# MachinaIO/mxx

Hardware: AMD Instinct MI355X
Metric: dcrt_ring_ops_per_s (higher is better)
Workload: dtype u32

## Files before the change

mxx_amd/csrc/arith.hip:

```cpp
#include "matmul_tile.h"

#include <algorithm>
#include <vector>

enum { OP_ADD = 0, OP_SUB = 1, OP_MUL = 2, OP_NEG = 3 };

template <typename W, int OP, bool BCAST, int VN>
__global__ void elementwise_kernel(W *__restrict__ out, const W *__restrict__ a, const W *__restrict__ b,
                                   const LimbConst *__restrict__ limbs, uint32_t L, uint32_t logN,
                                   size_t words_per_poly, size_t total_vecs) {
    size_t v = static_cast<size_t>(blockIdx.x) * blockDim.x + threadIdx.x;
    const size_t stride = static_cast<size_t>(gridDim.x) * blockDim.x;
    for (; v < total_vecs; v += stride) {
        const size_t w0 = v * VN;
        const uint32_t limb = static_cast<uint32_t>((w0 >> logN) % L);
        const LimbConst lc = limbs[limb];
        const W q = static_cast<W>(lc.q);
        const size_t bw0 = BCAST ? (w0 % words_per_poly) : w0;
        W av[VN], bv[VN], ov[VN];
        if (VN == 1) {
            av[0] = a[w0];
            bv[0] = b[bw0];
        } else {
            typedef typename std::conditional<sizeof(W) == 4, uint4, ulonglong2>::type V16;
// ... 322 lines not shown
        if (pending + kMmKC > lazy) {
            pending = 0;
#pragma unroll
            for (int i = 0; i < 8; ++i)
#pragma unroll
                for (int j = 0; j < 8; ++j) acc[i][j] = reduce_u64_sum(acc[i][j], q, lc.mu64);
        }
        if (ch + 1 < nchunks) stage(buf ^ 1);
        __syncthreads();
    }
#pragma unroll
    for (int i = 0; i < 8; ++i) {
        const uint32_t r = r0 + wr * 8 + i;
        if (r >= rows) continue;
#pragma unroll
        for (int j = 0; j < 8; ++j) {
            const uint32_t c = c0 + wc * 8 + j;
            if (c >= cols) continue;
            C[(static_cast<size_t>(r) * cols + c) * polyw + base] = reduce_u64_sum(acc[i][j], q, lc.mu64);
        }
    }
}

static int launch_matmul_lds_u32(GpuMatrix *out, const GpuMatrix *lhs, const GpuMatrix *rhs) {
    GpuContext *ctx = out->ctx;
    const uint32_t rows = static_cast<uint32_t>(lhs->rows), inner = static_cast<uint32_t>(lhs->cols),
                   cols = static_cast<uint32_t>(rhs->cols);
    const uint32_t L = static_cast<uint32_t>(matrix_limbs(out)), N = static_cast<uint32_t>(ctx->N);
    const uint32_t row_tiles = (rows + 15) / 16, col_tiles = (cols + 15) / 16, slot_chunks = N / 64;
    const uint64_t groups = static_cast<uint64_t>(L) * slot_chunks;
    const uint64_t blocks = groups * row_tiles * col_tiles;
    if (blocks > 0x7fffffffull) return set_error("gpu_matrix_mul: matrix too large");
    const uint32_t remap = (groups % 8 == 0) ? 1u : 0u;
    ctx->last_kernel = "matmul_lds_kernel_u32 (64 slots x 16x16 tile, operands staged through registers into LDS)";
    MXX_LAUNCH(matmul_lds_kernel_u32, dim3(static_cast<unsigned>(blocks)), dim3(256), 0, ctx->stream,
                       static_cast<uint32_t *>(words_ptr(out)), static_cast<const uint32_t *>(words_ptr(lhs)),
                       static_cast<const uint32_t *>(words_ptr(rhs)), ctx->d_limbs, rows, inner, cols, L, N, row_tiles,
                       col_tiles, slot_chunks, remap);
    HIP_TRY(hipGetLastError());
    return 0;
}

template <typename W, int TR, int TC, int SV, bool PF = false>
static int launch_matmul_cfg(GpuMatrix *out, const GpuMatrix *lhs, const GpuMatrix *rhs) {
    GpuContext *ctx = out->ctx;
    const uint32_t rows = static_cast<uint32_t>(lhs->rows), inner = static_cast<uint32_t>(lhs->cols),
                   cols = static_cast<uint32_t>(rhs->cols);
    const uint32_t L = static_cast<uint32_t>(matrix_limbs(out)), N = static_cast<uint32_t>(ctx->N);
    if (!tile_grid_fits(rows, cols, TR, TC)) return set_error("gpu_matrix_mul: matrix too large");
    const TileGrid g = tile_grid<TR, TC, SV>(ctx, rows, cols, L, rhs->bytes);
    const bool nt = g.streamed;
    auto label = [](bool nt_, int pk) {
        return std::string("matmul_kernel<") + (sizeof(W) == 4 ? "u32," : "u64,") + std::to_string(TR) + "," + std::to_string(TC) + "," +
               std::to_string(SV) + (PF ? ",loads-ahead" : "") + (nt_ ? ",nt" : "") +
               (pk == 2 ? ",packed24 B" : pk == 1 ? ",packed24 A" : "") +
               "> (register tile rows x cols x slots per lane" + (nt_ ? ", B streamed once with non-temporal loads" : "") +
               (pk ? ", 3-byte residues" : "") + ")";
    };
    static const std::string name[2][3] = {{label(false, 0), label(false, 1), label(false, 2)}, {label(true, 0), label(true, 1), label(true, 2)}};
    W *c = static_cast<W *>(words_ptr(out));
#define MXX_MM(NT, PK) \
    MXX_LAUNCH((matmul_kernel<W, TR, TC, SV, PF, NT, PK>), g.grid, dim3(g.threads), 0, ctx->stream, c, a, b, ctx->d_limbs, rows, inner, cols, L, N, g.col_tiles)
    if constexpr (sizeof(W) == 4 && SV == 4) {
        if (lhs->ctx == ctx && rhs->ctx == ctx) {
            if (lhs->layout.v.load(std::memory_order_acquire) == GPU_MATRIX_LAYOUT_PACKED24 &&
                rhs->layout.v.load(std::memory_order_acquire) == GPU_MATRIX_LAYOUT_PACKED24)
                (void)words_ptr(lhs);
            std::lock_guard<std::mutex> lk(ctx->layout_mutex);
            bool pa = false, pb = false;
            const W *a = static_cast<const W *>(packed24_ptr(lhs, &pa)), *b = static_cast<const W *>(packed24_ptr(rhs, &pb));
            if (pa && pb) return set_error("gpu_matrix_mul: both operands packed");
            const int pk = (pa ? 1 : 0) | (pb ? 2 : 0);
            ctx->last_kernel = name[nt ? 1 : 0][pk].c_str();
            switch (pk | (nt ? 4 : 0)) {
                case 0: MXX_MM(false, 0); break;
                case 1: MXX_MM(false, 1); break;
                case 2: MXX_MM(false, 2); break;
                case 4: MXX_MM(true, 0); break;
                case 5: MXX_MM(true, 1); break;
                default: MXX_MM(true, 2); break;
            }
            HIP_TRY(hipGetLastError());
            return 0;
        }
    }
    const W *a = static_cast<const W *>(words_ptr(lhs)), *b = static_cast<const W *>(words_ptr(rhs));
    ctx->last_kernel = name[nt ? 1 : 0][0].c_str();
    if (nt) MXX_MM(true, 0);
    else MXX_MM(false, 0);
#undef MXX_MM
    HIP_TRY(hipGetLastError());
    return 0;
}

int launch_matmul(GpuMatrix *out, const GpuMatrix *lhs, const GpuMatrix *rhs) {
    GpuContext *ctx = out->ctx;
    const size_t rows = lhs->rows, cols = rhs->cols;
    const int N = ctx->N;
    if (ctx->wide)
        return dispatch_stacked_tile(ctx, stacked_tile(ctx, rows, cols, matrix_limbs(out)), [&](auto cfg) {
            typedef decltype(cfg) T;
            return launch_matmul_cfg<typename T::W, T::TR, T::TC, T::SV>(out, lhs, rhs);
        });
    {
        const char force = ctx->env.matmul_path;
        const bool lds_ok = N >= 64 && (N % 64) == 0;
        const bool want_mfma = force ? (force == 'm') : false;
        if (want_mfma) {
            const int rc = launch_matmul_mfma_u32(out, lhs, rhs);
            if (rc >= 0) return rc;
        }
        const size_t inner = lhs->cols;
        const bool narrow = cols < 16 && inner < 128;
        const bool rows32 = !narrow && rows >= 24 && (rows % 32 == 0 || rows % 32 >= 24);
        const bool want_wide = force ? (force == 'w') : (rows32 && cols >= 32 && ((cols + 31) / 32) * 2 <= (cols + 15) / 16);
        if (want_wide) {
            const int rc = launch_matmul_dma32_u32(out, lhs, rhs);
            if (rc >= 0) return rc;
        }
        const bool want_dma = force ? (force == 'd' || force == 'w') : (rows32 && cols >= 16);
        if (want_dma) {
            const int rc = launch_matmul_dma_u32(out, lhs, rhs);
            if (rc >= 0) return rc;
        }
        const uint64_t lds_blocks = static_cast<uint64_t>(matrix_limbs(out)) * (N / 64) * ((cols + 15) / 16);
        const bool thin = rows <= 2 && cols >= 8 &&
                          lds_blocks <= 512 && (inner >= 128 || (rows >= 2 && inner >= 64));
        const bool want_lds = force ? (force == 'l' || force == 'd' || force == 'w') : ((rows >= 9 && cols >= 8 && !narrow) || thin);
        if (lds_ok && want_lds) return launch_matmul_lds_u32(out, lhs, rhs);
    }
    if (N >= 4) {
        switch (ctx->env.matmul_tile) {
#define MXX_TILE(R, C, S)                                                                   \
    case (R * 100 + C * 10 + S) * 2: return launch_matmul_cfg<uint32_t, R, C, S>(out, lhs, rhs); \
    case (R * 100 + C * 10 + S) * 2 + 1: return launch_matmul_cfg<uint32_t, R, C, S, true>(out, lhs, rhs);
            MXX_TILE(1, 8, 4) MXX_TILE(1, 4, 4) MXX_TILE(2, 8, 4) MXX_TILE(2, 4, 4) MXX_TILE(3, 4, 4) MXX_TILE(4, 4, 4)
            MXX_TILE(3, 8, 2) MXX_TILE(4, 8, 1) MXX_TILE(8, 8, 1) MXX_TILE(4, 8, 2)
#undef MXX_TILE
            default: break;
        }
        if (rows > 4 && rows <= 8) return launch_matmul_cfg<uint32_t, 8, 8, 1>(out, lhs, rhs);
        if (rows >= 4) {
            const uint64_t waves4 = static_cast<uint64_t>((N + 63) / 64) * ((cols + 7) / 8) * matrix_limbs(out);
            return waves4 <= 8192 ? launch_matmul_cfg<uint32_t, 4, 8, 1, true>(out, lhs, rhs) : launch_matmul_cfg<uint32_t, 4, 8, 1>(out, lhs, rhs);
        }
        if (rows == 3) {
            const uint64_t waves3 = static_cast<uint64_t>((N / 4 + 63) / 64) * ((cols + 3) / 4) * matrix_limbs(out);
            return waves3 <= 4096 ? launch_matmul_cfg<uint32_t, 3, 4, 4, true>(out, lhs, rhs) : launch_matmul_cfg<uint32_t, 3, 4, 4>(out, lhs, rhs);
        }
        const uint32_t tc = (rows >= 2 || cols >= 8) ? 8 : 4;
        const uint64_t tile_waves = static_cast<uint64_t>((N / 4 + 63) / 64) * ((rows + 1) / 2) * ((cols + tc - 1) / tc) * matrix_limbs(out);
        const bool ahead = tile_waves <= (rows >= 2 ? 1024u : 8192u);
        if (rows >= 2) return ahead ? launch_matmul_cfg<uint32_t, 2, 8, 4, true>(out, lhs, rhs) : launch_matmul_cfg<uint32_t, 2, 8, 4>(out, lhs, rhs);
        if (cols >= 8) return ahead ? launch_matmul_cfg<uint32_t, 1, 8, 4, true>(out, lhs, rhs) : launch_matmul_cfg<uint32_t, 1, 8, 4>(out, lhs, rhs);
        return ahead ? launch_matmul_cfg<uint32_t, 1, 4, 4, true>(out, lhs, rhs) : launch_matmul_cfg<uint32_t, 1, 4, 4>(out, lhs, rhs);
    }
    return launch_matmul_cfg<uint32_t, 1, 4, 1>(out, lhs, rhs);
}

template <typename W, int OP, bool BCAST>
static int launch_elementwise_typed(GpuMatrix *out, const GpuMatrix *a, const GpuMatrix *b) {
    GpuContext *ctx = out->ctx;
    const size_t words = matrix_words(out);
    if (words == 0) return 0;
    const size_t wpp = matrix_limbs(out) * static_cast<size_t>(ctx->N);
    const uint32_t L = static_cast<uint32_t>(matrix_limbs(out));
    constexpr int VNATIVE = 16 / sizeof(W);
    MXX_TRACE_BYTES(static_cast<double>(words) * sizeof(W) * (1 + (OP == OP_NEG || BCAST || a == b ? 1 : 2)));
    if (ctx->N >= VNATIVE) {
        const size_t vecs = words / VNATIVE;
        unsigned blocks = static_cast<unsigned>(std::min<size_t>((vecs + 255) / 256, 16384));
        MXX_LAUNCH((elementwise_kernel<W, OP, BCAST, VNATIVE>), dim3(blocks), dim3(256), 0, ctx->stream,
                           static_cast<W *>(words_ptr(out)), static_cast<const W *>(words_ptr(a)),
                           static_cast<const W *>(words_ptr(b)), ctx->d_limbs, L, ctx->logN, wpp, vecs);
    } else {
        unsigned blocks = static_cast<unsigned>(std::min<size_t>((words + 255) / 256, 16384));
        MXX_LAUNCH((elementwise_kernel<W, OP, BCAST, 1>), dim3(blocks), dim3(256), 0, ctx->stream,
                           static_cast<W *>(words_ptr(out)), static_cast<const W *>(words_ptr(a)),
                           static_cast<const W *>(words_ptr(b)), ctx->d_limbs, L, ctx->logN, wpp, words);
    }
    HIP_TRY(hipGetLastError());
    return 0;
}

template <int OP, bool BCAST>
static int launch_elementwise(GpuMatrix *out, const GpuMatrix *a, const GpuMatrix *b) {
    if (ctx_activate(out->ctx)) return 1;
    return out->ctx->wide ? launch_elementwise_typed<uint64_t, OP, BCAST>(out, a, b)
                          : launch_elementwise_typed<uint32_t, OP, BCAST>(out, a, b);
}

static GpuMatrix matrix_view(const GpuMatrix *m, size_t first_poly, size_t rows, size_t cols, size_t poly_bytes) {
    GpuMatrix v;
    v.ctx = m->ctx;
    v.level = m->level;
    v.rows = rows;
    v.cols = cols;
    v.format = m->format;
    v.storage = static_cast<char *>(words_ptr(m)) + first_poly * poly_bytes;
    v.bytes = rows * cols * poly_bytes;
    return v;
}

extern "C" int gpupoly_matrix_add_rows(GpuMatrix *out, size_t dst_row, const GpuMatrix *lhs, const GpuMatrix *rhs) {
    ABI_GUARD_BEGIN
    if (!out || !lhs || !rhs) return set_error("gpupoly_matrix_add_rows: null matrix");
    if (matrix_check_same_shape(lhs, rhs, "gpupoly_matrix_add_rows")) return 1;
    if (out->ctx != lhs->ctx || out->level != lhs->level) return set_error("gpupoly_matrix_add_rows: context/level mismatch");
    if (out->cols != lhs->cols || dst_row > out->rows || lhs->rows > out->rows - dst_row)
        return set_error("gpupoly_matrix_add_rows: row block out of range");
    if (lhs->format != rhs->format) return set_error("gpupoly_matrix_add_rows: operands must share a format");
    if (row_block_overlaps(out, dst_row, lhs->rows, lhs) || row_block_overlaps(out, dst_row, lhs->rows, rhs))
        return set_error("gpupoly_matrix_add_rows: output must not alias an input");
    const size_t poly_bytes = matrix_limbs(out) * static_cast<size_t>(out->ctx->N) * out->ctx->word_bytes;
    GpuMatrix view = matrix_view(out, dst_row * out->cols, lhs->rows, lhs->cols, poly_bytes);
    int rc = launch_elementwise<OP_ADD, false>(&view, lhs, rhs);
    if (rc) return rc;
    out->format = lhs->format;
    return 0;
    ABI_GUARD_END
}

extern "C" int gpupoly_matrix_ntt_add_rows(GpuMatrix *out, size_t dst_row, GpuMatrix *coeff, const GpuMatrix *addend,
                                           int consume_coeff) {
    ABI_GUARD_BEGIN
    if (!out || !coeff || !addend) return set_error("gpupoly_matrix_ntt_add_rows: null matrix");
    if (matrix_check_same_shape(coeff, addend, "gpupoly_matrix_ntt_add_rows")) return 1;
    if (out->ctx != coeff->ctx || out->level != coeff->level) return set_error("gpupoly_matrix_ntt_add_rows: context/level mismatch");
    if (out->cols != coeff->cols || dst_row > out->rows || coeff->rows > out->rows - dst_row)
        return set_error("gpupoly_matrix_ntt_add_rows: row block out of range");
    if (coeff->format != GPU_POLY_FORMAT_COEFF || addend->format != GPU_POLY_FORMAT_EVAL)
        return set_error("gpupoly_matrix_ntt_add_rows: expects a COEFF matrix and an EVAL addend");
    if (row_block_overlaps(out, dst_row, coeff->rows, coeff) || row_block_overlaps(out, dst_row, coeff->rows, addend))
        return set_error("gpupoly_matrix_ntt_add_rows: output must not alias an input");
    GpuContext *ctx = out->ctx;
    out->format = GPU_POLY_FORMAT_EVAL;
    const size_t polys = matrix_polys(coeff);
    if (polys == 0) return 0;
    if (ctx_activate(ctx)) return 1;
    const size_t L = matrix_limbs(out);
    const size_t poly_bytes = L * static_cast<size_t>(ctx->N) * ctx->word_bytes;
    GpuMatrix view = matrix_view(out, dst_row * out->cols, coeff->rows, coeff->cols, poly_bytes);
    view.format = GPU_POLY_FORMAT_EVAL;
    if (!ctx->wide) {
        const int rc = launch_ntt_add_u32(ctx, static_cast<uint32_t *>(words_ptr(&view)), static_cast<const uint32_t *>(words_ptr(coeff)),
                                          static_cast<const uint32_t *>(words_ptr(addend)), polys * L, static_cast<uint32_t>(L));
        if (rc >= 0) return rc;
    }
    if (consume_coeff) {
        int rc = launch_ntt(ctx, words_ptr(coeff), polys * L, static_cast<int>(L), false);
        if (rc) return rc;
        coeff->format = GPU_POLY_FORMAT_EVAL;
        return launch_elementwise<OP_ADD, false>(&view, coeff, addend);
    }
    MXX_TRACED_COPY("copy (device to device)", ctx->stream, 2.0 * view.bytes,
                    HIP_TRY(hipMemcpyAsync(words_ptr(&view), words_ptr(coeff), view.bytes, hipMemcpyDeviceToDevice, ctx->stream)));
    int rc = launch_ntt(ctx, words_ptr(&view), polys * L, static_cast<int>(L), false);
    if (rc) return rc;
    return launch_elementwise<OP_ADD, false>(&view, &view, addend);
    ABI_GUARD_END
}

extern "C" int gpu_matrix_add(GpuMatrix *out, const GpuMatrix *lhs, const GpuMatrix *rhs) {
    ABI_GUARD_BEGIN
    if (matrix_check_same_shape(out, lhs, "gpu_matrix_add") || matrix_check_same_shape(lhs, rhs, "gpu_matrix_add"))
        return 1;
    if (partial_overlap(out, lhs) || partial_overlap(out, rhs))
        return set_error("gpu_matrix_add: the output overlaps an operand without being the same block");
    int rc = launch_elementwise<OP_ADD, false>(out, lhs, rhs);
    if (rc) return rc;
    out->format = rhs->format;
    return 0;
    ABI_GUARD_END
}

extern "C" int gpu_matrix_sub(GpuMatrix *out, const GpuMatrix *lhs, const GpuMatrix *rhs) {
    ABI_GUARD_BEGIN
    if (matrix_check_same_shape(out, lhs, "gpu_matrix_sub") || matrix_check_same_shape(lhs, rhs, "gpu_matrix_sub"))
        return 1;
    if (partial_overlap(out, lhs) || partial_overlap(out, rhs))
        return set_error("gpu_matrix_sub: the output overlaps an operand without being the same block");
    int rc = launch_elementwise<OP_SUB, false>(out, lhs, rhs);
    if (rc) return rc;
    out->format = rhs->format;
    return 0;
    ABI_GUARD_END
}

extern "C" int gpupoly_matrix_neg(GpuMatrix *out, const GpuMatrix *src) {
    ABI_GUARD_BEGIN
    if (matrix_check_same_shape(out, src, "gpupoly_matrix_neg")) return 1;
    if (partial_overlap(out, src))
        return set_error("gpupoly_matrix_neg: the output overlaps the source without being the same block");
    int rc = launch_elementwise<OP_NEG, false>(out, src, src);
    if (rc) return rc;
    out->format = src->format;
    return 0;
    ABI_GUARD_END
}

extern "C" int gpu_matrix_mul_scalar(GpuMatrix *out, const GpuMatrix *lhs, const GpuMatrix *scalar) {
    ABI_GUARD_BEGIN
    if (!scalar) return set_error("gpu_matrix_mul_scalar: null scalar");
    if (matrix_check_same_shape(out, lhs, "gpu_matrix_mul_scalar")) return 1;
    if (scalar->ctx != lhs->ctx || scalar->level != lhs->level)
        return set_error("gpu_matrix_mul_scalar: context/level mismatch");
// ... 501 lines not shown
```

mxx_amd/csrc/common.h:

```cpp
#pragma once

#include <hip/hip_runtime.h>

#include <atomic>
#include <cstddef>
#include <cstdint>
#include <cstdio>
#include <exception>
#include <map>
#include <unordered_map>
#include <mutex>
#include <string>
#include <vector>

#include "../../include/gpupoly.h"

constexpr size_t GPUPOLY_MAX_LIMBS = 64;

struct LimbConst {
    uint64_t q;
    uint64_t mu;
    uint64_t mu64;
    uint64_t n_inv;
    uint64_t n_inv_sh;
    uint64_t mu32;
    uint64_t inv_last_w;
    uint64_t inv_last_w_sh;
    uint32_t kbits;
    uint32_t lazy_terms;
};

struct EnvSwitches {
    int ntt_path = 0;
    int ntt14 = 0;
    bool decompose_fused = true;
    char matmul_path = 0;
    int matmul_tile = 0;
    bool gsamp_simple = false;
    bool gsamp_no_uni = false;
    bool p1_simple = false;
    int sampler_per_lane = 0;
    int sampler_fill_every = 0;
    bool ntt64_int = false;
    int ntt_phase = 0;
    bool serde_general = false;
    bool rng_compat = false;
    bool pack24 = true;
    size_t mul_decompose_many_budget = 0;
    size_t gadget_scalar_budget = 0;
    char mul_sum_path = 0;
    void load();
};

struct GpuContext {
    EnvSwitches env;
    int device = 0;
    std::vector<int> gpu_ids;
    uint32_t logN = 0;
    int N = 0;
    int level = 0;
    uint32_t dnum = 0;
    int limb_count = 0;
    bool wide = false;
    int word_bytes = 4;
    uint32_t crt_bits = 0;
    std::vector<uint64_t> moduli;
    hipStream_t stream = nullptr;
    LimbConst *d_limbs = nullptr;
    LimbConst *d_limbs_r = nullptr;
    void *d_tw_fwd = nullptr;
    void *d_tw_fwd_sh = nullptr;
    void *d_tw_inv = nullptr;
    void *d_tw_inv_sh = nullptr;
    void *d_tw2_fwd = nullptr;
    void *d_tw2_inv = nullptr;
    bool lazy_ok = false;
    bool tight_ok = false;
    void *d_tw2s_inv = nullptr;
    bool signed_ok = false;
    void *d_twf_fwd = nullptr, *d_twf_inv = nullptr;
    void *d_flimbs = nullptr;
    bool f64_ok = false;
    uint64_t *d_garner = nullptr;
    std::vector<uint64_t> garner_inv;
    std::vector<LimbConst> limbs;
    hipEvent_t timer_start = nullptr, timer_stop = nullptr;
    std::vector<hipEvent_t> marks;
    std::mutex mutex;
    bool pool_ok = false;
    std::mutex alloc_mutex;
    std::multimap<size_t, void *> free_blocks;
    std::unordered_map<void *, size_t> live_blocks;
    size_t cached_bytes = 0, cache_limit = 0;
    std::atomic<const char *> last_kernel{""};
    bool pack24_ok = false;
    std::mutex layout_mutex;
    std::map<uint32_t, void *> gadget_weights;
    std::map<std::vector<uint64_t>, void *> gadget_const_tables;
};

struct LayoutTag {
    std::atomic<int> v{GPU_MATRIX_LAYOUT_WORDS};
    LayoutTag() = default;
    LayoutTag(const LayoutTag &o) : v(o.v.load(std::memory_order_acquire)) {}
    LayoutTag &operator=(const LayoutTag &o) {
        v.store(o.v.load(std::memory_order_acquire), std::memory_order_release);
        return *this;
    }
};

struct GpuMatrix {
    GpuContext *ctx = nullptr;
    int level = 0;
    size_t rows = 0, cols = 0;
    int format = GPU_POLY_FORMAT_EVAL;
    void *storage = nullptr;
    size_t bytes = 0;
    LayoutTag layout;
    bool borrowed = false;
    GpuMatrix *parent = nullptr;
    int views = 0;
};

struct GpuEventSet {
    std::vector<hipEvent_t> events;
    int device = 0;
    void *staging = nullptr;
    GpuContext *ctx = nullptr;
    void *dev_staging = nullptr;
};

struct GpuP1CovarianceCache {
    GpuContext *ctx = nullptr;
    int level = 0;
    size_t d = 0, m = 0, n = 0;
    double sigma = 0, s = 0, dgg_stddev = 0;
    double *sqrt_var = nullptr;
    double *update_coeff = nullptr;
    void *karney_div = nullptr;
};

static inline dim3 item_grid(size_t items, unsigned threads) {
    const size_t blocks = (items + threads - 1) / threads;
    const size_t max_x = (static_cast<size_t>(1) << 31) / threads;
    if (blocks <= max_x) return dim3(static_cast<unsigned>(blocks ? blocks : 1));
    const size_t y = (blocks + max_x - 1) / max_x;
    return dim3(static_cast<unsigned>((blocks + y - 1) / y), static_cast<unsigned>(y));
}
#if defined(__HIPCC__)
__device__ __forceinline__ size_t item_index() {
    return (static_cast<size_t>(blockIdx.y) * gridDim.x + blockIdx.x) * blockDim.x + threadIdx.x;
}
#endif

extern std::atomic<uint64_t> g_kernel_launches;
extern std::atomic<int> g_trace_on;
void trace_launch_begin(const char *name, hipStream_t stream, dim3 grid, dim3 block);
void trace_launch_end(hipStream_t stream);
void trace_set_bytes(double bytes);
#define MXX_TRACE_BYTES(b)                                                                        \
    do {                                                                                          \
        if (g_trace_on.load(std::memory_order_relaxed)) trace_set_bytes(static_cast<double>(b)); \
    } while (0)
#define MXX_LAUNCH(kern, grid, block, lds, strm, ...)                          \
    do {                                                                       \
        g_kernel_launches.fetch_add(1, std::memory_order_relaxed);             \
        const bool mxx_tr_ = g_trace_on.load(std::memory_order_relaxed) != 0;  \
        if (mxx_tr_) trace_launch_begin(#kern, strm, grid, block);             \
        hipLaunchKernelGGL(kern, grid, block, lds, strm, __VA_ARGS__);         \
        if (mxx_tr_) trace_launch_end(strm);                                   \
    } while (0)
#define MXX_TRACED_COPY(name, strm, bytes, stmt)                               \
    do {                                                                       \
        const bool mxx_tr_ = g_trace_on.load(std::memory_order_relaxed) != 0;  \
        if (mxx_tr_) {                                                         \
            trace_set_bytes(static_cast<double>(bytes));                       \
            trace_launch_begin(name, strm, dim3(0), dim3(0));                  \
        }                                                                      \
        stmt;                                                                  \
        if (mxx_tr_) trace_launch_end(strm);                                   \
    } while (0)

int set_error(const char *msg);
int set_error(const std::string &msg);
int set_error(hipError_t err, const char *what);

#define HIP_TRY(expr)                                          \
    do {                                                       \
        hipError_t _e = (expr);                                \
        if (_e != hipSuccess) return set_error(_e, #expr);     \
    } while (0)

extern int (*g_roctx_push)(const char *);
extern int (*g_roctx_pop)();
void roctx_init_once();
struct RoctxScope {
    bool on;
    explicit RoctxScope(const char *name) {
        roctx_init_once();
        on = g_roctx_push != nullptr;
        if (on) g_roctx_push(name);
    }
    ~RoctxScope() {
        if (on) g_roctx_pop();
    }
};

#define ABI_GUARD_BEGIN try { RoctxScope roctx_scope_(__func__);
#define ABI_GUARD_END                                                         \
    }                                                                         \
    catch (const std::exception &e) { return set_error(e.what()); }           \
    catch (...) { return set_error("unknown exception in libgpupoly"); }

inline size_t matrix_polys(const GpuMatrix *m) { return m->rows * m->cols; }
inline size_t matrix_limbs(const GpuMatrix *m) { return static_cast<size_t>(m->level) + 1; }
inline size_t matrix_words(const GpuMatrix *m) { return matrix_polys(m) * matrix_limbs(m) * static_cast<size_t>(m->ctx->N); }

void *words_ptr(const GpuMatrix *m);
const void *packed24_ptr(const GpuMatrix *m, bool *packed);
inline size_t packed24_bytes(const GpuMatrix *m) { return m->bytes / 4 * 3; }
inline bool storage_overlaps(const GpuMatrix *x, const GpuMatrix *y) {
    if (x == y) return true;
    if (!x->storage || !y->storage || x->bytes == 0 || y->bytes == 0) return false;
    const size_t xb = x->layout.v.load(std::memory_order_acquire) == GPU_MATRIX_LAYOUT_PACKED24 ? packed24_bytes(x) : x->bytes;
    const size_t yb = y->layout.v.load(std::memory_order_acquire) == GPU_MATRIX_LAYOUT_PACKED24 ? packed24_bytes(y) : y->bytes;
    const char *xs = static_cast<const char *>(x->storage), *ys = static_cast<const char *>(y->storage);
    return xs < ys + yb && ys < xs + xb;
}
inline bool same_block(const GpuMatrix *x, const GpuMatrix *y) {
    return x == y || (x->storage == y->storage && x->bytes == y->bytes);
}
inline bool partial_overlap(const GpuMatrix *out, const GpuMatrix *operand) {
    return storage_overlaps(out, operand) && !same_block(out, operand);
}
inline bool row_block_overlaps(const GpuMatrix *m, size_t row, size_t rows, const GpuMatrix *y) {
    if (m->layout.v.load(std::memory_order_acquire) == GPU_MATRIX_LAYOUT_PACKED24) return rows && m->cols && storage_overlaps(m, y);
    if (!m->storage) return false;
    const size_t poly_bytes = matrix_limbs(m) * static_cast<size_t>(m->ctx->N) * m->ctx->word_bytes;
    GpuMatrix block;
    block.storage = static_cast<char *>(m->storage) + row * m->cols * poly_bytes;
    block.bytes = rows * m->cols * poly_bytes;
    return storage_overlaps(&block, y);
}
bool pack24_eligible(const GpuMatrix *m);
int pack24_store(GpuMatrix *m, bool ntt);

int sample_impl(GpuMatrix *out, int dist, double sigma, GpuRngSeed seed, size_t full_ncol, size_t col_offset, bool keep_coeff,
                size_t row_offset = 0, uint32_t tower_first = 0, uint32_t tower_count = 0);

int ctx_activate(const GpuContext *ctx);
bool ctx_is_registered(const GpuContext *ctx);
int ctx_alloc(GpuContext *ctx, size_t bytes, void **out);
void ctx_free(GpuContext *ctx, void *ptr);
struct CtxBlock {
    GpuContext *ctx;
    void *ptr = nullptr;
    explicit CtxBlock(GpuContext *c) : ctx(c) {}
    CtxBlock(const CtxBlock &) = delete;
    CtxBlock &operator=(const CtxBlock &) = delete;
    ~CtxBlock() {
        if (ptr) ctx_free(ctx, ptr);
    }
    int alloc(size_t bytes) { return ctx_alloc(ctx, bytes, &ptr); }
    void *release() {
        void *p = ptr;
        ptr = nullptr;
        return p;
    }
};
int matrix_check_same_shape(const GpuMatrix *a, const GpuMatrix *b, const char *who);
int coeff_domain_source(const GpuMatrix *mat, CtxBlock &scratch, const void **src);

int launch_ntt(GpuContext *ctx, void *data, size_t vectors, int limbs_per_poly, bool inverse);
int launch_ntt_lds_u32(GpuContext *ctx, uint32_t *data, size_t vectors, uint32_t L, bool inverse);
int launch_ntt_digits_u32(GpuContext *ctx, uint32_t *out, const uint32_t *coeff, size_t out_vectors, uint32_t L,
                          uint32_t src_cols, uint32_t towers, uint32_t dpt, uint32_t base_bits, size_t k, uint32_t td0 = 0);
int launch_ntt_lds_u64(GpuContext *ctx, uint64_t *data, size_t vectors, uint32_t L, bool inverse);
int launch_ntt_digits_u64(GpuContext *ctx, uint64_t *out, const uint64_t *coeff, size_t out_vectors, uint32_t L,
                          uint32_t src_cols, uint32_t towers, uint32_t dpt, uint32_t base_bits, size_t k, uint32_t td0 = 0);
int launch_intt_oop_u32(GpuContext *ctx, uint32_t *out, const uint32_t *in, size_t vectors, uint32_t L);
int launch_ntt_add_u32(GpuContext *ctx, uint32_t *out, const uint32_t *src, const uint32_t *add, size_t vectors, uint32_t L);
int launch_mul_intt_u32(GpuContext *ctx, uint32_t *out, const uint32_t *in, const uint32_t *w, size_t vectors, uint32_t L);
int launch_matmul(GpuMatrix *out, const GpuMatrix *lhs, const GpuMatrix *rhs);
int launch_ntt_fwd_pack24_u32(GpuContext *ctx, uint32_t *out, const uint32_t *in, size_t vectors, uint32_t L);
int launch_matmul_dma_u32(GpuMatrix *out, const GpuMatrix *lhs, const GpuMatrix *rhs);
int launch_matmul_dma32_u32(GpuMatrix *out, const GpuMatrix *lhs, const GpuMatrix *rhs);
int launch_matmul_mfma_u32(GpuMatrix *out, const GpuMatrix *lhs, const GpuMatrix *rhs);
int launch_copy_block(GpuMatrix *out, const GpuMatrix *src, size_t dst_row, size_t dst_col, size_t src_row,
                      size_t src_col, size_t rows, size_t cols, bool add);
int launch_scatter_i64(GpuMatrix *out, const int64_t *vals);
```

mxx_amd/csrc/runtime.hip:

```cpp
#include "common.h"

#include <algorithm>
#include <cstdlib>
#include <iterator>
#include <map>
#include <cstring>
#include <dlfcn.h>

typedef unsigned __int128 u128h;

static thread_local std::string g_last_error;

int set_error(const char *msg) {
    g_last_error = msg ? msg : "unknown error";
    return 1;
}
int set_error(const std::string &msg) {
    g_last_error = msg;
    return 1;
}
int set_error(hipError_t err, const char *what) {
    g_last_error = std::string(what ? what : "hip call") + ": " + hipGetErrorString(err);
    (void)hipGetLastError();
    return 1;
// ... 86 lines not shown
extern "C" int gpupoly_trace_begin(void) {
    ABI_GUARD_BEGIN
    std::lock_guard<std::mutex> lk(g_trace_mutex);
    for (const TraceEntry &en : g_trace) {
        trace_event_return(en.device, en.e0);
        trace_event_return(en.device, en.e1);
    }
    g_trace.clear();
    g_trace_on.store(1, std::memory_order_relaxed);
    return 0;
    ABI_GUARD_END
}

extern "C" const char *gpupoly_trace_end(void) {
    try {
        g_trace_on.store(0, std::memory_order_relaxed);
        std::lock_guard<std::mutex> lk(g_trace_mutex);
        g_trace_report.clear();
        int prev = 0;
        (void)hipGetDevice(&prev);
        char line[512];
        for (const TraceEntry &en : g_trace) {
            if (!en.closed) continue;
            (void)hipSetDevice(en.device);
            float ms = 0;
            hipError_t e = hipEventSynchronize(en.e1);
            if (e == hipSuccess) e = hipEventElapsedTime(&ms, en.e0, en.e1);
            if (e != hipSuccess) {
                (void)hipSetDevice(prev);
                set_error(e, "gpupoly_trace_end: hipEventElapsedTime");
                return nullptr;
            }
            std::snprintf(line, sizeof line, "%s\t%llu\t%u\t%.0f\t%.6f\n", en.name, en.blocks, en.threads, en.bytes, ms);
            g_trace_report += line;
        }
        for (const TraceEntry &en : g_trace) {
            trace_event_return(en.device, en.e0);
            trace_event_return(en.device, en.e1);
        }
        g_trace.clear();
        (void)hipSetDevice(prev);
        return g_trace_report.c_str();
    } catch (...) {
        set_error("gpupoly_trace_end: exception");
        return nullptr;
    }
}

int (*g_roctx_push)(const char *) = nullptr;
int (*g_roctx_pop)() = nullptr;
void roctx_init_once() {
    static std::once_flag once;
    std::call_once(once, [] {
        const char *sw = std::getenv("MXX_HIP_ROCTX");
        const bool profiled = std::getenv("ROCP_TOOL_LIBRARIES") != nullptr || std::getenv("ROCPROFILER_REGISTER_FORCE_LOAD") != nullptr;
        if (sw ? sw[0] == '0' : !profiled) return;
        for (const char *name : {"librocprofiler-sdk-roctx.so.1", "librocprofiler-sdk-roctx.so", "libroctx64.so.4", "libroctx64.so"}) {
            void *h = dlopen(name, RTLD_NOW | RTLD_GLOBAL);
            if (!h) continue;
            auto push = reinterpret_cast<int (*)(const char *)>(dlsym(h, "roctxRangePushA"));
            auto pop = reinterpret_cast<int (*)()>(dlsym(h, "roctxRangePop"));
            if (push && pop) {
                g_roctx_pop = pop;
                g_roctx_push = push;
                return;
            }
        }
    });
}

static inline uint64_t h_mulmod(uint64_t a, uint64_t b, uint64_t q) { return (uint64_t)(((u128h)a * b) % q); }
static uint64_t h_powmod(uint64_t b, uint64_t e, uint64_t q) {
    uint64_t r = 1 % q;
    b %= q;
    while (e) {
        if (e & 1) r = h_mulmod(r, b, q);
        b = h_mulmod(b, b, q);
        e >>= 1;
    }
    return r;
}
static uint64_t h_invmod_prime(uint64_t a, uint64_t q) { return h_powmod(a % q, q - 2, q); }

static bool h_is_prime(uint64_t n) {
    static const uint64_t bases[] = {2, 3, 5, 7, 11, 13, 17, 19, 23, 29, 31, 37};
    if (n < 2) return false;
    for (uint64_t b : bases)
        if (n % b == 0) return n == b;
    uint64_t d = n - 1;
    int s = 0;
    while (!(d & 1)) { d >>= 1; ++s; }
    for (uint64_t b : bases) {
        uint64_t x = h_powmod(b, d, n);
        if (x == 1 || x == n - 1) continue;
        bool comp = true;
        for (int r = 1; r < s; ++r) {
            x = h_mulmod(x, x, n);
            if (x == n - 1) { comp = false; break; }
        }
        if (comp) return false;
    }
    return true;
}

static uint64_t h_min_primitive_root(uint64_t q, uint64_t order) {
    uint64_t qm1 = q - 1;
    int v = __builtin_ctzll(qm1);
    int want = __builtin_ctzll(order);
    uint64_t odd = qm1 >> v;
    uint64_t maximal = 0;
    for (uint64_t x = 2; x < q; ++x) {
        uint64_t r = h_powmod(x, odd, q);
        if (h_powmod(r, 1ull << (v - 1), q) != 1) { maximal = r; break; }
    }
    uint64_t root = h_powmod(maximal, 1ull << (v - want), q);
    uint64_t sq = h_mulmod(root, root, q);
    uint64_t cur = root, best = root;
    for (uint64_t i = 1; i < order / 2; ++i) {
        cur = h_mulmod(cur, sq, q);
        if (cur < best) best = cur;
    }
    return best;
}

static inline uint32_t h_bitrev(uint32_t x, uint32_t bits) {
    uint32_t r = 0;
    for (uint32_t i = 0; i < bits; ++i) { r = (r << 1) | (x & 1); x >>= 1; }
    return r;
}
static inline uint32_t h_bits(uint64_t v) { return v ? 64 - (uint32_t)__builtin_clzll(v) : 0; }

void EnvSwitches::load() {
    *this = EnvSwitches();
    if (const char *e = std::getenv("MXX_HIP_NTT_PATH")) {
        if (e[0] == 'l') ntt_path = 1;
        else if (e[0] == 'g' && e[1] == 'e') ntt_path = 2;
        else if (e[0] == 'g' && e[1] == 'l') ntt_path = 3;
    }
    if (const char *e = std::getenv("MXX_HIP_NTT14")) ntt14 = e[0] == 'w' ? 1 : (e[0] == 'u' ? 2 : 0);
    if (const char *e = std::getenv("MXX_HIP_DECOMPOSE_FUSED")) decompose_fused = e[0] != '0';
    if (const char *e = std::getenv("MXX_HIP_MATMUL_PATH")) matmul_path = e[0];
    if (const char *e = std::getenv("MXX_HIP_MATMUL_TILE")) {
        if (e[0] && e[1] && e[2]) matmul_tile = ((e[0] - '0') * 100 + (e[1] - '0') * 10 + (e[2] - '0')) * 2 + (e[3] == 'p');
    }
    if (const char *e = std::getenv("MXX_HIP_GSAMP")) {
        gsamp_simple = e[0] == 's';
        gsamp_no_uni = e[0] == 'n';
    }
    if (const char *e = std::getenv("MXX_HIP_P1")) p1_simple = e[0] == 's';
    if (const char *e = std::getenv("MXX_HIP_NTT64")) ntt64_int = e[0] == 'i';
    if (const char *e = std::getenv("MXX_HIP_RNG_COMPAT")) rng_compat = e[0] == 'r';
    if (const char *e = std::getenv("MXX_HIP_SERDE")) serde_general = e[0] == 'g';
    if (const char *e = std::getenv("MXX_HIP_PACK24")) pack24 = !(std::strcmp(e, "0") == 0 || std::strcmp(e, "off") == 0);
    if (const char *e = std::getenv("MXX_HIP_MUL_DECOMPOSE_MANY_BUDGET")) mul_decompose_many_budget = static_cast<size_t>(std::strtoull(e, nullptr, 10));
    if (const char *e = std::getenv("MXX_HIP_GADGET_SCALAR_BUDGET")) gadget_scalar_budget = static_cast<size_t>(std::strtoull(e, nullptr, 10));
    if (const char *e = std::getenv("MXX_HIP_MUL_SUM_PATH")) mul_sum_path = (e[0] == 't' || e[0] == 's') ? e[0] : 0;
    if (const char *e = std::getenv("MXX_HIP_SAMPLER_PER_LANE")) {
        const int v = std::atoi(e);
        if (v >= 1 && v <= 4096) sampler_per_lane = v;
    }
    if (const char *e = std::getenv("MXX_HIP_NTT_PHASE")) {
        const int v = std::atoi(e);
        if (v >= 0 && v <= 127) ntt_phase = v;
    }
    if (const char *e = std::getenv("MXX_HIP_SAMPLER_FILL_EVERY")) {
        const int v = std::atoi(e);
        if (v >= 1 && v <= 8) sampler_fill_every = v;
    }
}

static std::mutex g_registry_mutex;
static std::vector<GpuContext *> g_contexts;
bool ctx_is_registered(const GpuContext *ctx) {
    std::lock_guard<std::mutex> lk(g_registry_mutex);
    return std::find(g_contexts.begin(), g_contexts.end(), ctx) != g_contexts.end();
}

extern "C" int gpupoly_reload_env(void) {
    std::lock_guard<std::mutex> lk(g_registry_mutex);
    for (GpuContext *c : g_contexts) c->env.load();
    return 0;
}

int ctx_activate(const GpuContext *ctx) {
    HIP_TRY(hipSetDevice(ctx->device));
    return 0;
}

static size_t round_block(size_t bytes) {
    const size_t gran = bytes >= (size_t(1) << 20) ? (size_t(1) << 20) : 4096;
    return (bytes + gran - 1) / gran * gran;
}

static void cache_trim(GpuContext *ctx, size_t limit) {
    while (ctx->cached_bytes > limit && !ctx->free_blocks.empty()) {
        auto it = std::prev(ctx->free_blocks.end());
        (void)hipFree(it->second);
        ctx->cached_bytes -= it->first;
        ctx->free_blocks.erase(it);
    }
}

int ctx_alloc(GpuContext *ctx, size_t bytes, void **out) {
    *out = nullptr;
    if (bytes == 0) return 0;
    const size_t want = round_block(bytes);
    std::lock_guard<std::mutex> lk(ctx->alloc_mutex);
    auto it = ctx->free_blocks.lower_bound(want);
    if (it != ctx->free_blocks.end() && it->first <= want + want / 4) {
        *out = it->second;
        ctx->live_blocks[*out] = it->first;
        ctx->cached_bytes -= it->first;
        ctx->free_blocks.erase(it);
        return 0;
    }
    hipError_t e = hipMalloc(out, want);
    if (e != hipSuccess) {
        (void)hipGetLastError();
        cache_trim(ctx, 0);
        e = hipMalloc(out, want);
    }
    if (e != hipSuccess) {
        (void)hipGetLastError();
        {
            std::lock_guard<std::mutex> reg(g_registry_mutex);
            for (GpuContext *other : g_contexts) {
                if (other == ctx || other->device != ctx->device) continue;
                if (!other->alloc_mutex.try_lock()) continue;
                cache_trim(other, 0);
                other->alloc_mutex.unlock();
            }
        }
        e = hipMalloc(out, want);
        if (e != hipSuccess) {
            *out = nullptr;
            return set_error(e, "hipMalloc");
        }
    }
    ctx->live_blocks[*out] = want;
    return 0;
}

void ctx_free(GpuContext *ctx, void *ptr) {
    if (!ptr) return;
    std::lock_guard<std::mutex> lk(ctx->alloc_mutex);
    auto it = ctx->live_blocks.find(ptr);
    if (it == ctx->live_blocks.end()) {
        (void)hipFree(ptr);
        return;
    }
    const size_t size = it->second;
    ctx->live_blocks.erase(it);
    if (!ctx->pool_ok) {
        (void)hipFree(ptr);
        return;
    }
    ctx->free_blocks.emplace(size, ptr);
    ctx->cached_bytes += size;
    cache_trim(ctx, ctx->cache_limit);
}

template <typename W>
static int upload_tables(GpuContext *ctx, const std::vector<std::vector<uint64_t>> &fwd,
                         const std::vector<std::vector<uint64_t>> &inv) {
    const size_t N = ctx->N, L = ctx->limb_count;
    const unsigned shift = sizeof(W) * 8;
    std::vector<W> h_f(L * N), h_fs(L * N), h_i(L * N), h_is(L * N);
    for (size_t l = 0; l < L; ++l) {
        uint64_t q = ctx->moduli[l];
        for (size_t j = 0; j < N; ++j) {
            h_f[l * N + j] = (W)fwd[l][j];
            h_fs[l * N + j] = (W)(((u128h)fwd[l][j] << shift) / q);
            h_i[l * N + j] = (W)inv[l][j];
            h_is[l * N + j] = (W)(((u128h)inv[l][j] << shift) / q);
        }
    }
    size_t bytes = L * N * sizeof(W);
    HIP_TRY(hipMalloc(&ctx->d_tw_fwd, bytes));
    HIP_TRY(hipMalloc(&ctx->d_tw_fwd_sh, bytes));
    HIP_TRY(hipMalloc(&ctx->d_tw_inv, bytes));
    HIP_TRY(hipMalloc(&ctx->d_tw_inv_sh, bytes));
    HIP_TRY(hipMemcpy(ctx->d_tw_fwd, h_f.data(), bytes, hipMemcpyHostToDevice));
    HIP_TRY(hipMemcpy(ctx->d_tw_fwd_sh, h_fs.data(), bytes, hipMemcpyHostToDevice));
    HIP_TRY(hipMemcpy(ctx->d_tw_inv, h_i.data(), bytes, hipMemcpyHostToDevice));
    HIP_TRY(hipMemcpy(ctx->d_tw_inv_sh, h_is.data(), bytes, hipMemcpyHostToDevice));
    std::vector<W> h_pf(2 * L * N), h_pi(2 * L * N);
    for (size_t i = 0; i < L * N; ++i) {
        h_pf[2 * i] = static_cast<W>(0) - h_f[i];
        h_pf[2 * i + 1] = h_fs[i];
        h_pi[2 * i] = h_i[i];
        h_pi[2 * i + 1] = h_is[i];
    }
    HIP_TRY(hipMalloc(&ctx->d_tw2_fwd, 2 * bytes));
    HIP_TRY(hipMalloc(&ctx->d_tw2_inv, 2 * bytes));
    HIP_TRY(hipMemcpy(ctx->d_tw2_fwd, h_pf.data(), 2 * bytes, hipMemcpyHostToDevice));
    HIP_TRY(hipMemcpy(ctx->d_tw2_inv, h_pi.data(), 2 * bytes, hipMemcpyHostToDevice));
    if (sizeof(W) == 8 && ctx->crt_bits <= 51 && N >= 2) {
        struct HostTwF { double w, wi; };
        struct HostF64Limb { double q, qinv; HostTwF n_inv, last_w; };
        std::vector<HostTwF> tf(L * N), ti(L * N);
        std::vector<HostF64Limb> fl(L);
        for (size_t l = 0; l < L; ++l) {
            const double qd = static_cast<double>(ctx->moduli[l]);
            for (size_t j = 0; j < N; ++j) {
                tf[l * N + j] = {static_cast<double>(fwd[l][j]), static_cast<double>(fwd[l][j]) / qd};
                ti[l * N + j] = {static_cast<double>(inv[l][j]), static_cast<double>(inv[l][j]) / qd};
// ... 388 lines not shown
```

Measured before the change: 7.362 million.

## Add skinny24 matmul kernel for single-row times packed24 RHS

Adds a dedicated kernel for 1-row-by-many-column matmuls whose right operand is stored in the 24-bit packed layout. It streams B once using non-temporal buffer loads of 12 bytes per lane, or 16-byte loads staged through a wave-private LDS slice, unpacks 3-byte residues and accumulates lazily. The aim is to cut memory traffic and improve coalescing for the bandwidth-bound skinny case. It only activates when B is packed24, the grid is streamed and not small, and it adds env knobs and an extra dispatch branch.

```diff
diff --git a/mxx_amd/csrc/arith.hip b/mxx_amd/csrc/arith.hip
--- a/mxx_amd/csrc/arith.hip
+++ b/mxx_amd/csrc/arith.hip
@@ -498,6 +498,10 @@
         const uint64_t tile_waves = static_cast<uint64_t>((N / 4 + 63) / 64) * ((rows + 1) / 2) * ((cols + tc - 1) / tc) * matrix_limbs(out);
         const bool ahead = tile_waves <= (rows >= 2 ? 1024u : 8192u);
         if (rows >= 2) return ahead ? launch_matmul_cfg<uint32_t, 2, 8, 4, true>(out, lhs, rhs) : launch_matmul_cfg<uint32_t, 2, 8, 4>(out, lhs, rhs);
+        if (cols >= 8) {
+            const int rc = launch_matmul_skinny24(out, lhs, rhs, ahead);
+            if (rc >= 0) return rc;
+        }
         if (cols >= 8) return ahead ? launch_matmul_cfg<uint32_t, 1, 8, 4, true>(out, lhs, rhs) : launch_matmul_cfg<uint32_t, 1, 8, 4>(out, lhs, rhs);
         return ahead ? launch_matmul_cfg<uint32_t, 1, 4, 4, true>(out, lhs, rhs) : launch_matmul_cfg<uint32_t, 1, 4, 4>(out, lhs, rhs);
     }
diff --git a/mxx_amd/csrc/common.h b/mxx_amd/csrc/common.h
--- a/mxx_amd/csrc/common.h
+++ b/mxx_amd/csrc/common.h
@@ -46,6 +46,8 @@
     bool serde_general = false;
     bool rng_compat = false;
     bool pack24 = true;
+    int skinny24 = 0;
+    int skinny24_shape = 0;
     size_t mul_decompose_many_budget = 0;
     size_t gadget_scalar_budget = 0;
     char mul_sum_path = 0;
@@ -283,6 +285,8 @@
 int launch_mul_intt_u32(GpuContext *ctx, uint32_t *out, const uint32_t *in, const uint32_t *w, size_t vectors, uint32_t L);
 int launch_matmul(GpuMatrix *out, const GpuMatrix *lhs, const GpuMatrix *rhs);
 int launch_ntt_fwd_pack24_u32(GpuContext *ctx, uint32_t *out, const uint32_t *in, size_t vectors, uint32_t L);
+int launch_matmul_skinny24(GpuMatrix *out, const GpuMatrix *lhs, const GpuMatrix *rhs, bool small_grid);
+int skinny24_parse_shape(const char *s);
 int launch_matmul_dma_u32(GpuMatrix *out, const GpuMatrix *lhs, const GpuMatrix *rhs);
 int launch_matmul_dma32_u32(GpuMatrix *out, const GpuMatrix *lhs, const GpuMatrix *rhs);
 int launch_matmul_mfma_u32(GpuMatrix *out, const GpuMatrix *lhs, const GpuMatrix *rhs);
diff --git a/mxx_amd/csrc/matmul_skinny24.hip b/mxx_amd/csrc/matmul_skinny24.hip
--- /dev/null
+++ b/mxx_amd/csrc/matmul_skinny24.hip
@@ -0,0 +1,185 @@
+#include "common.h"
+#include "matmul_tile.h"
+#include "modarith.h"
+
+#include <map>
+#include <string>
+
+namespace skinny24 {
+
+typedef uint32_t u32x3 __attribute__((ext_vector_type(3)));
+typedef uint32_t u32x4 __attribute__((ext_vector_type(4)));
+
+__device__ __forceinline__ __amdgpu_buffer_rsrc_t row_rsrc(const char *base, uint32_t bytes) {
+    return __builtin_amdgcn_make_buffer_rsrc(const_cast<char *>(base), 0, static_cast<int>(bytes), 0x00020000);
+}
+constexpr int kAuxNT = 2;
+
+__device__ __forceinline__ void unpack4(uint32_t w0, uint32_t w1, uint32_t w2, uint32_t *o) {
+    o[0] = w0 & 0xffffffu;
+    o[1] = __builtin_amdgcn_alignbit(w1, w0, 24) & 0xffffffu;
+    o[2] = __builtin_amdgcn_alignbit(w2, w1, 16) & 0xffffffu;
+    o[3] = w2 >> 8;
+}
+
+template <int TC, int G, int WPE, int MAP>
+__global__ void __launch_bounds__(256, WPE)
+    kernel(uint32_t *__restrict__ C, const uint32_t *__restrict__ A, const uint32_t *__restrict__ B, const LimbConst *__restrict__ limbs,
+           uint32_t inner, uint32_t cols, uint32_t L, uint32_t N) {
+    static_assert((TC == 8 || TC == 4) && TC % G == 0 && (MAP == 12 || MAP == 16), "skinny24 shape");
+    const uint32_t limb = blockIdx.z, c0 = blockIdx.y * TC;
+    const uint32_t i = (blockIdx.x * blockDim.x + threadIdx.x) * 4;
+    if (i >= N) return;
+    const LimbConst lc = limbs[limb];
+    const uint32_t q = static_cast<uint32_t>(lc.q);
+
+    uint32_t bcol[TC];
+#pragma unroll
+    for (int c = 0; c < TC; ++c) bcol[c] = ((min(c0 + c, cols - 1)) * L + limb) * N * 3;
+    const uint32_t bstep = cols * L * N * 3;
+    const char *bk = reinterpret_cast<const char *>(B);
+    const char *arow = reinterpret_cast<const char *>(A) + static_cast<size_t>(limb) * N * 4;
+    const size_t astep = static_cast<size_t>(L) * N * 4;
+    const uint32_t a_off = i * 4;
+    const uint32_t lane = threadIdx.x & 63u;
+    const uint32_t b_off = MAP == 12 ? i * 3 : (lane < 48 ? (i - lane * 4) * 3 + lane * 16 : bstep);
+    __shared__ u32x4 stage[MAP == 16 ? 4 : 1][MAP == 16 ? G : 1][64];
+    const uint32_t wave = threadIdx.x >> 6;
+
+    uint64_t acc[TC][4];
+#pragma unroll
+    for (int c = 0; c < TC; ++c)
+#pragma unroll
+        for (int s = 0; s < 4; ++s) acc[c][s] = 0;
+    const uint32_t lazy = lc.lazy_terms;
+    uint32_t pending = 0;
+    for (uint32_t k = 0; k < inner; ++k) {
+        const u32x4 av = __builtin_amdgcn_raw_buffer_load_b128(row_rsrc(arow, N * 4), a_off, 0, 0);
+        arow += astep;
+#pragma unroll
+        for (int g0 = 0; g0 < TC; g0 += G) {
+            uint32_t raw[G][3];
+            if constexpr (MAP == 12) {
+#pragma unroll
+                for (int g = 0; g < G; ++g) {
+                    const u32x3 t = __builtin_amdgcn_raw_buffer_load_b96(row_rsrc(bk, bstep), b_off, bcol[g0 + g], kAuxNT);
+                    raw[g][0] = t[0];
+                    raw[g][1] = t[1];
+                    raw[g][2] = t[2];
+                }
+            } else {
+                __builtin_amdgcn_wave_barrier();
+                u32x4 t[G];
+#pragma unroll
+                for (int g = 0; g < G; ++g) t[g] = __builtin_amdgcn_raw_buffer_load_b128(row_rsrc(bk, bstep), b_off, bcol[g0 + g], kAuxNT);
+#pragma unroll
+                for (int g = 0; g < G; ++g) stage[wave][g][lane] = t[g];
+                __builtin_amdgcn_wave_barrier();
+#pragma unroll
+                for (int g = 0; g < G; ++g) {
+                    const uint32_t *p = reinterpret_cast<const uint32_t *>(&stage[wave][g][0]) + lane * 3;
+                    raw[g][0] = p[0];
+                    raw[g][1] = p[1];
+                    raw[g][2] = p[2];
+                }
+            }
+#pragma unroll
+            for (int g = 0; g < G; ++g) {
+                uint32_t bv[4];
+                unpack4(raw[g][0], raw[g][1], raw[g][2], bv);
+#pragma unroll
+                for (int s = 0; s < 4; ++s) acc[g0 + g][s] += static_cast<uint64_t>(av[s]) * static_cast<uint64_t>(bv[s]);
+            }
+        }
+        bk += bstep;
+        if (++pending == lazy) {
+            pending = 0;
+#pragma unroll
+            for (int c = 0; c < TC; ++c)
+#pragma unroll
+                for (int s = 0; s < 4; ++s) acc[c][s] = reduce_u64_sum(acc[c][s], q, lc.mu64);
+        }
+    }
+#pragma unroll
+    for (int c = 0; c < TC; ++c) {
+        if (c0 + c >= cols) continue;
+        u32x4 o;
+#pragma unroll
+        for (int s = 0; s < 4; ++s) o[s] = reduce_u64_sum(acc[c][s], q, lc.mu64);
+        *reinterpret_cast<u32x4 *>(C + (static_cast<size_t>(c0 + c) * L + limb) * N + i) = o;
+    }
+}
+
+#define MXX_SKINNY24_SHAPES(X)                                          \
+    X(8, 1, 5, 12) X(8, 2, 5, 12) X(8, 4, 5, 12) X(8, 8, 5, 12) X(8, 8, 4, 12)  \
+    X(8, 1, 5, 16) X(8, 2, 5, 16) X(8, 4, 5, 16)                        \
+    X(4, 1, 8, 12) X(4, 2, 8, 12) X(4, 4, 8, 12) X(4, 1, 8, 16) X(4, 2, 8, 16) X(4, 4, 8, 16)
+
+constexpr int shape_key(int tc, int g, int wpe, int map) { return ((tc * 16 + g) * 16 + wpe) * 32 + map; }
+
+}
+
+int skinny24_parse_shape(const char *s) {
+    int v[4] = {0, 0, 0, 0};
+    for (int f = 0; f < 4; ++f) {
+        if (*s < '0' || *s > '9') return 0;
+        while (*s >= '0' && *s <= '9' && v[f] < 100) v[f] = v[f] * 10 + (*s++ - '0');
+        if (f < 3 && *s++ != ',') return 0;
+    }
+    if (*s || v[0] > 15 || v[1] > 15 || v[2] > 15 || v[3] > 31) return 0;
+    return skinny24::shape_key(v[0], v[1], v[2], v[3]);
+}
+
+static constexpr int kSkinny24Default = skinny24::shape_key(8, 2, 5, 12);
+
+int launch_matmul_skinny24(GpuMatrix *out, const GpuMatrix *lhs, const GpuMatrix *rhs, bool small_grid) {
+    using namespace skinny24;
+    GpuContext *ctx = out->ctx;
+    const EnvSwitches &env = ctx->env;
+    if (env.skinny24 == 1 || ctx->wide || lhs->ctx != ctx || rhs->ctx != ctx) return -1;
+    const uint32_t inner = static_cast<uint32_t>(lhs->cols), cols = static_cast<uint32_t>(rhs->cols);
+    const uint32_t L = static_cast<uint32_t>(matrix_limbs(out)), N = static_cast<uint32_t>(ctx->N);
+    if (lhs->rows != 1 || cols < 8 || N < 4) return -1;
+    if (static_cast<uint64_t>(cols) * L * N * 3 >= 0xfffffff0ull) return -1;
+    if (rhs->layout.v.load(std::memory_order_acquire) != GPU_MATRIX_LAYOUT_PACKED24) return -1;
+    const bool force = env.skinny24 == 2;
+    int key = force && env.skinny24_shape ? env.skinny24_shape : kSkinny24Default;
+    const int tc = key / (16 * 16 * 32);
+    const TileGrid g = tc == 4 ? tile_grid<1, 4, 4>(ctx, 1, cols, L, rhs->bytes) : tile_grid<1, 8, 4>(ctx, 1, cols, L, rhs->bytes);
+    if (!force && (!g.streamed || small_grid)) return -1;
+    if (!tile_grid_fits(1, cols, 1, tc == 4 ? 4 : 8)) return set_error("gpu_matrix_mul: matrix too large");
+    const bool fell_back = key % 32 == 16 && N % 256 != 0;
+    if (fell_back) key = key - 16 + 12;
+    uint32_t *c = static_cast<uint32_t *>(words_ptr(out));
+    if (lhs->layout.v.load(std::memory_order_acquire) == GPU_MATRIX_LAYOUT_PACKED24) (void)words_ptr(lhs);
+    std::lock_guard<std::mutex> lk(ctx->layout_mutex);
+    bool pa = false, pb = false;
+    const uint32_t *a = static_cast<const uint32_t *>(packed24_ptr(lhs, &pa)), *b = static_cast<const uint32_t *>(packed24_ptr(rhs, &pb));
+    if (pa || !pb) return -1;
+    const char *label;
+    {
+        static std::mutex label_mutex;
+        static std::map<int, std::string> labels;
+        std::lock_guard<std::mutex> ll(label_mutex);
+        std::string &s = labels[key * 2 + (fell_back ? 1 : 0)];
+        if (s.empty())
+            s = "skinny24::kernel<TC=" + std::to_string(tc) + ",G=" + std::to_string(key / (16 * 32) % 16) + ",WPE=" + std::to_string(key / 32 % 16) +
+                ",MAP=" + std::to_string(key % 32) + (fell_back ? " (16 asked: partial wave)" : "") +
+                ",nt,packed24 B> (the tile of matmul_kernel<u32,1," + std::to_string(tc) + ",4,nt,packed24 B>, one row x TC columns x 4 slots per lane, " +
+                "B streamed once with non-temporal loads, 3-byte residues, " +
+                (key % 32 == 16 ? "16-byte requests through a wave-private LDS slice" : "12 bytes per lane") + ")";
+        label = s.c_str();
+    }
+    switch (key) {
+#define MXX_SKINNY24_CASE(TC_, G_, WPE_, MAP_)                                                                                               \
+    case shape_key(TC_, G_, WPE_, MAP_):                                                                                                     \
+        MXX_LAUNCH((kernel<TC_, G_, WPE_, MAP_>), g.grid, dim3(g.threads), 0, ctx->stream, c, a, b, ctx->d_limbs, inner, cols, L, N); \
+        break;
+        MXX_SKINNY24_SHAPES(MXX_SKINNY24_CASE)
+#undef MXX_SKINNY24_CASE
+        default: return set_error("gpu_matrix_mul: MXX_HIP_SKINNY24 names a shape that is not instantiated");
+    }
+    ctx->last_kernel = label;
+    HIP_TRY(hipGetLastError());
+    return 0;
+}
diff --git a/mxx_amd/csrc/runtime.hip b/mxx_amd/csrc/runtime.hip
--- a/mxx_amd/csrc/runtime.hip
+++ b/mxx_amd/csrc/runtime.hip
@@ -262,6 +262,13 @@
     if (const char *e = std::getenv("MXX_HIP_RNG_COMPAT")) rng_compat = e[0] == 'r';
     if (const char *e = std::getenv("MXX_HIP_SERDE")) serde_general = e[0] == 'g';
     if (const char *e = std::getenv("MXX_HIP_PACK24")) pack24 = !(std::strcmp(e, "0") == 0 || std::strcmp(e, "off") == 0);
+    if (const char *e = std::getenv("MXX_HIP_SKINNY24")) {
+        if (std::strcmp(e, "0") == 0) skinny24 = 1;
+        else if (std::strncmp(e, "force", 5) == 0 && (e[5] == 0 || e[5] == ':')) {
+            skinny24 = 2;
+            if (e[5] == ':') skinny24_shape = skinny24_parse_shape(e + 6) ? skinny24_parse_shape(e + 6) : -1;
+        }
+    }
     if (const char *e = std::getenv("MXX_HIP_MUL_DECOMPOSE_MANY_BUDGET")) mul_decompose_many_budget = static_cast<size_t>(std::strtoull(e, nullptr, 10));
     if (const char *e = std::getenv("MXX_HIP_GADGET_SCALAR_BUDGET")) gadget_scalar_budget = static_cast<size_t>(std::strtoull(e, nullptr, 10));
     if (const char *e = std::getenv("MXX_HIP_MUL_SUM_PATH")) mul_sum_path = (e[0] == 't' || e[0] == 's') ? e[0] : 0;
```

Result: faster. 8.016 million, median of 6 (+8.9%).
